# eldenpark/halo2-pse

Hardware: AMD Instinct MI355X
Metric: bn254_msm_g1_adds_per_sec (higher is better)
Workload: dtype u32x8 (256-bit Montgomery integers)

## Files before the change

halo2-pse_amd/__init__.py:

```python
import ctypes
import os
import subprocess

import numpy as np

_HERE = os.path.dirname(os.path.abspath(__file__))
LIB_PATH = os.environ.get("HALO2_HIP_LIB") or os.path.join(_HERE, "libhalo2hip.so")
HEADER_PATH = os.path.join(os.path.dirname(_HERE), "include", "halo2hip.h")

_lib = None


class H2HipError(RuntimeError):
    pass


def build(force=False, jobs=4):
    args = ["make", "-C", _HERE, "-j%d" % jobs]
    if force:
        args.append("-B")
    subprocess.check_call(args, stdout=subprocess.DEVNULL)
    return LIB_PATH


# ... 1140 lines not shown
                                                         ctypes.c_uint32(domain.extended_k), _p(domain.extended_omega), _p(domain.g_coset),
                                                         _p(domain.g_coset_inv), ctypes.c_uint32(blinding_factors), _dptr(d_l0), _dptr(d_l_last),
                                                         _dptr(d_l_active_row), _stream()), "h2hip_key_lagrange_columns_bn254_device")


def set_keygen_group(group_bytes=0):
    _check(lib().h2hip_debug_set_keygen_group(ctypes.c_uint64(group_bytes)), "h2hip_debug_set_keygen_group")


def gen_scalars_device(seed, n, start=0, device="cuda"):
    import torch
    out = torch.empty((n, 4), dtype=torch.int64, device=device)
    _check(lib().h2hip_gen_scalars_device(ctypes.c_uint64(seed), ctypes.c_uint64(start), ctypes.c_size_t(n), _dptr(out), _stream()),
           "h2hip_gen_scalars_device")
    return out


def gen_points_device(seed, n, start=0, device="cuda"):
    import torch
    out = torch.empty((n, 8), dtype=torch.int64, device=device)
    _check(lib().h2hip_gen_points_device(ctypes.c_uint64(seed), ctypes.c_uint64(start), ctypes.c_size_t(n), _dptr(out), _stream()),
           "h2hip_gen_points_device")
    return out


def to_numpy_u64(t):
    return t.detach().cpu().numpy().view(np.uint64)


def set_msm_window(c):
    _check(lib().h2hip_set_msm_window(ctypes.c_uint32(c)), "h2hip_set_msm_window")


def get_msm_window(n):
    return int(lib().h2hip_get_msm_window(n))


def get_msm_window_fixed_base(n):
    return int(lib().h2hip_get_msm_window_fixed_base(n))


def msm_min_n():
    return int(lib().h2hip_msm_min_n())


def ntt_min_log_n():
    return int(lib().h2hip_ntt_min_log_n())


def lazy_pin_after():
    return int(lib().h2hip_lazy_pin_after())


def profile_enable(on=True):
    _check(lib().h2hip_profile_enable(int(on)), "h2hip_profile_enable")


def profile_reset():
    _check(lib().h2hip_profile_reset(), "h2hip_profile_reset")


def profile_get(stage):
    ms = ctypes.c_double(0)
    cnt = ctypes.c_uint64(0)
    _check(lib().h2hip_profile_get(stage.encode(), ctypes.byref(ms), ctypes.byref(cnt)), "h2hip_profile_get")
    return ms.value, cnt.value
# ... 1 lines not shown
```

halo2-pse_amd/csrc/engine.h:

```cpp
#pragma once
#include <hip/hip_runtime.h>
#include <stdint.h>
#include <stdio.h>
#include <string.h>

#include <map>
#include <mutex>
#include <shared_mutex>
#include <string>
#include <vector>

#include "../../include/halo2hip.h"
#include "ecu.h"

namespace h2 {

void set_error(const char* fmt, ...);

#define H2_CHECK(expr)                                                                             \
    do {                                                                                           \
        hipError_t _e = (expr);                                                                    \
        if (_e != hipSuccess) {                                                                    \
            h2::set_error("%s:%d: %s -> %s", __FILE__, __LINE__, #expr, hipGetErrorString(_e));    \
            return 2;                                                                              \
// ... 321 lines not shown
int kzg_setup_device(Ctx* c, uint32_t k, const Fe& s, Affine* d_g, Affine* d_gl, hipStream_t stream);

const Fe* pinned_column_lookup(Ctx* c, const uint64_t* h_col, size_t elems);

void evalh_debug_set_max_local_slots(uint32_t v);
void evalh_debug_set_lookup_group_bytes(uint64_t v);
int evalh_debug_compile_stats(const h2hip_graph* g, uint32_t* n_ops, uint32_t* n_slots);
int evalh_debug_program_muls(const h2hip_graph* g, uint32_t* n_mul);
void evalh_debug_set_codegen(int mode, uint32_t max_ops);
void evalh_debug_codegen_stats(uint64_t out[5]);
int evalh_debug_codegen_source(const h2hip_graph* g, char* buf, size_t cap, size_t* len, int compile, double* seconds, size_t* code_bytes);
void evalh_modules_free(Ctx* c);
void evalh_rtc_shutdown();
int evaluate_h_validate(const h2hip_evalh_desc* d, const void* values);
int evaluate_h_host(Ctx* c, const h2hip_evalh_desc* d, uint64_t* values, bool dev, hipStream_t s);
int lookup_compress_validate(uint32_t n_fixed, uint32_t n_advice, uint32_t n_instance, uint32_t n_challenges, const h2hip_graph* graphs,
                             size_t n_graphs);
int lookup_compress_device(Ctx* c, uint32_t k, const Fe* const* fixed, uint32_t n_fixed, const Fe* const* advice, uint32_t n_advice,
                           const Fe* const* instance, uint32_t n_instance, const uint64_t* challenges, uint32_t n_challenges,
                           const uint64_t theta[4], const h2hip_graph* graphs, size_t n_graphs, Fe* const* out, hipStream_t s);
int check_gates_validate(uint32_t n_fixed, uint32_t n_advice, uint32_t n_instance, uint32_t n_challenges, const h2hip_graph* graphs,
                         size_t n_graphs);
int check_gates_enqueue(Ctx* c, uint32_t k, const Fe* const* fixed, uint32_t n_fixed, const Fe* const* advice, uint32_t n_advice,
                        const Fe* const* instance, uint32_t n_instance, const uint64_t* challenges, uint32_t n_challenges,
                        const h2hip_graph* graphs, size_t n_graphs, uint64_t* d_mask, uint32_t words, hipStream_t s);

void msm_set_fuse_small(bool on);
void msm_set_window(uint32_t c);
void msm_set_max_chunk(size_t m);
void msm_set_stream(uint32_t chunks, double ratio, size_t min_n);
size_t msm_debug_ladder(size_t n, uint32_t chunks, double ratio, bool with_bases, size_t* out, size_t cap);
void msm_set_heavy_div(size_t d);
void msm_set_bin_entries(size_t d);
void msm_set_split_records(bool on);
void msm_set_bucket_order(int local);
void msm_set_quad_tail(bool on);
void msm_set_split_buckets(bool on);
void msm_set_plane_tail(bool on);
void msm_set_fuse_limits(size_t entries, size_t max_n);
void msm_set_rowcol(uint64_t lanes, uint32_t flavour);
void msm_set_reserved_cus(uint32_t k);
uint32_t msm_get_reserved_cus();
uint32_t msm_get_window(size_t n);
int msm_device(Ctx* c, const Fe* d_scalars, const Affine* d_bases, size_t n, XYZZ* h_out, hipStream_t s, const MsmTable* tab = nullptr);
int msm_batch_device(Ctx* c, const Fe* const* scalars, bool scalars_on_host, const Affine* d_bases, size_t n, size_t count, XYZZ* h_out,
                     hipStream_t s, const MsmTable* tab = nullptr, const Affine* h_bases = nullptr);
uint32_t msm_table_window(size_t n);
int msm_table_build(Ctx* c, const Affine* d_points, size_t n, uint32_t cw, Affine* d_table, hipStream_t s);

}
```

halo2-pse_amd/csrc/msm.hip:

```cpp
#include <hip/hip_ext.h>
#include <string.h>

#include <atomic>
#include <condition_variable>
#include <thread>
#include <vector>

#include "ecq.h"
#include "engine.h"
#include "host64.h"

namespace h2 {

#define MSM_MAX_C1 1024u
#define MSM_MAX_L 12u
#define MSM_STAGE 16384u
#define MSM_COUNT_TILE 4096u

struct MsmPlan {
    uint32_t c;
    uint32_t W;
    uint32_t q;
    uint32_t cb;
    uint32_t NB;
    uint32_t shared;
    uint32_t heavy_t;
    uint32_t chunk;
};

template <class F>
__device__ __forceinline__ void for_each_digit(const Fe& s, uint32_t c, uint32_t q, uint32_t W, F&& f) {
    uint64_t buf = 0;
    uint32_t nb = 0, w = 0, carry = 0;
    uint32_t width = q ? c : c - 1;
    auto emit = [&]() {
        uint32_t d = ((uint32_t)buf & ((1u << width) - 1)) + carry;
        uint32_t neg = 0;
        carry = 0;
        if (d > (1u << (width - 1))) {
            d = (1u << width) - d;
            neg = 1;
            carry = 1;
        }
        if (d) f(w, d - 1, neg);
        w++;
        buf >>= width;
        nb = nb > width ? nb - width : 0;
        width = w < q ? c : c - 1;
    };
#pragma unroll
    for (int limb = 0; limb < 8; limb++) {
        buf |= (uint64_t)s.l[limb] << nb;
        nb += 32;
        while (nb >= width && w < W) emit();
    }
    while (w < W) emit();
}

struct L1Args {
    const Fe* scalars_one;
    const Fe* const* list;
    uint32_t n, c, q, W, cb, L, C1;
    uint32_t shared, stride;
    uint32_t tile;
    uint16_t* tile_hist;
    const uint32_t* tile_off;
    uint2* tmp;
    uint32_t* tmp_e;
    uint16_t* tmp_k;
    const Affine* chk_bases;
    const Affine* chk_samples;
    uint32_t* chk_flag;
    size_t chk_n, chk_total;
};

__device__ __forceinline__ Fe fr_to_canonical(const Fe& x) {
    Fu c32 = fu_zero();
    c32.l[0] = 32;
    return fu_mul_canon<FrU>(fu_slice(x), c32);
}

#define MSM_TCHUNK 64u
#ifndef MSM_SCATTER_XG
#define MSM_SCATTER_XG 4u
#endif

__global__ void __launch_bounds__(256) msm_l1_count_kernel(L1Args a) {
    __shared__ uint32_t lh[MSM_MAX_C1];
    if (a.chk_flag && blockIdx.x == 0 && blockIdx.y == 0 && threadIdx.x < 4 * H2_PIN_SAMPLES) {
        const uint32_t k = threadIdx.x >> 2, part = threadIdx.x & 3;
        const size_t idx = pin_sample_index(a.chk_total, k);
        if (idx < a.chk_n) {
            const uint4 u = reinterpret_cast<const uint4*>(&a.chk_bases[idx])[part], v = reinterpret_cast<const uint4*>(&a.chk_samples[k])[part];
            if (u.x != v.x || u.y != v.y || u.z != v.z || u.w != v.w) atomicOr(a.chk_flag, 1u);
        }
    }
    for (uint32_t b = threadIdx.x; b < a.C1; b += 256) lh[b] = 0;
    __syncthreads();
    const Fe* __restrict__ scalars = a.list ? a.list[blockIdx.y] : a.scalars_one;
    const uint32_t set0 = a.shared ? blockIdx.y : blockIdx.y * a.W;
    for (uint32_t t = threadIdx.x; t < a.tile; t += 256) {
        const uint32_t i = blockIdx.x * a.tile + t;
        if (i < a.n) {
            const Fe sc = fr_to_canonical(scalars[i]);
            for_each_digit(sc, a.c, a.q, a.W, [&](uint32_t w, uint32_t slot, uint32_t) {
                const uint32_t gb = ((set0 + (a.shared ? 0u : w)) << a.cb) | slot;
                atomicAdd(&lh[gb >> a.L], 1u);
            });
        }
    }
    __syncthreads();
    uint16_t* row = a.tile_hist + (size_t)(blockIdx.y * gridDim.x + blockIdx.x) * a.C1;
    for (uint32_t b = threadIdx.x; b < a.C1; b += 256) row[b] = (uint16_t)lh[b];
}

__global__ void __launch_bounds__(256) msm_l1_chunk_kernel(const uint16_t* __restrict__ tile_hist, uint32_t n_tiles, uint32_t C1,
                                                           uint32_t* __restrict__ chunk_sum) {
    const uint32_t b = blockIdx.y * 256 + threadIdx.x;
    if (b >= C1) return;
    const uint32_t t0 = blockIdx.x * MSM_TCHUNK, t1 = t0 + MSM_TCHUNK < n_tiles ? t0 + MSM_TCHUNK : n_tiles;
    uint32_t sum = 0;
#pragma unroll 8
    for (uint32_t t = t0; t < t1; t++) sum += tile_hist[(size_t)t * C1 + b];
    chunk_sum[(size_t)blockIdx.x * C1 + b] = sum;
}

template <int BS>
__device__ __forceinline__ uint32_t block_scan_base(const uint32_t* cnt, uint32_t n, uint32_t per, uint32_t* ps, uint32_t* total) {
    const uint32_t t = threadIdx.x;
    uint32_t sum = 0;
    for (uint32_t j = 0; j < per; j++) {
        const uint32_t k = t * per + j;
        if (k < n) sum += cnt[k];
    }
    uint32_t inc = sum;
#pragma unroll
    for (uint32_t off = 1; off < 64; off <<= 1) {
        const uint32_t up = __shfl_up(inc, off, 64);
        if ((t & 63) >= off) inc += up;
    }
    if ((t & 63) == 63) ps[t >> 6] = inc;
    __syncthreads();
    uint32_t before = 0, all = 0;
#pragma unroll
    for (uint32_t w = 0; w < BS / 64; w++) {
        const uint32_t v = ps[w];
        if (w < (t >> 6)) before += v;
        all += v;
    }
    __syncthreads();
    *total = all;
    return before + inc - sum;
}

template <bool SPLIT>
__global__ void __launch_bounds__(1024) msm_l1_scatter_kernel(L1Args a) {
    __shared__ uint2 stage[MSM_STAGE];
    __shared__ uint32_t cur[MSM_MAX_C1];
    __shared__ uint32_t delta[MSM_MAX_C1];
    __shared__ uint32_t ps[16];
    constexpr uint32_t XG = MSM_SCATTER_XG;
    uint32_t tx = blockIdx.x;
    if (XG && tx < (gridDim.x & ~((8u << XG) - 1))) {
        const uint32_t q = tx >> (3 + XG), r = tx & ((8u << XG) - 1);
        tx = ((q * 8 + (r & 7)) << XG) | (r >> 3);
    }
    const size_t row = (size_t)(blockIdx.y * gridDim.x + tx) * a.C1;
    for (uint32_t b = threadIdx.x; b < a.C1; b += 1024) cur[b] = a.tile_hist[row + b];
    const Fe* __restrict__ scalars = a.list ? a.list[blockIdx.y] : a.scalars_one;
    const uint32_t set0 = a.shared ? blockIdx.y : blockIdx.y * a.W;
    const uint32_t i = tx * a.tile + threadIdx.x;
    const bool live = threadIdx.x < a.tile && i < a.n;
    Fe sc;
    if (live) sc = fr_to_canonical(scalars[i]);
    __syncthreads();
    uint32_t total;
    uint32_t run = block_scan_base<1024>(cur, a.C1, 1, ps, &total);
    if (threadIdx.x < a.C1) {
        const uint32_t b = threadIdx.x;
        delta[b] = a.tile_off[row + b] - run;
        cur[b] = run;
    }
    __syncthreads();
    if (live) {
        for_each_digit(sc, a.c, a.q, a.W, [&](uint32_t w, uint32_t slot, uint32_t neg) {
            const uint32_t gb = ((set0 + (a.shared ? 0u : w)) << a.cb) | slot;
            const uint32_t pos = atomicAdd(&cur[gb >> a.L], 1u);
            stage[pos] = make_uint2((a.shared ? w * a.stride + i : i) | (neg << 31), gb);
        });
    }
    __syncthreads();
    for (uint32_t pos = threadIdx.x; pos < total; pos += 1024) {
        const uint2 e = stage[pos];
        const uint32_t at = pos + delta[e.y >> a.L];
        if (SPLIT) {
            a.tmp_e[at] = e.x;
            a.tmp_k[at] = (uint16_t)(e.y & ((1u << a.L) - 1));
        } else {
            a.tmp[at] = e;
        }
    }
}

__global__ void __launch_bounds__(1024) msm_l1_scan_kernel(uint32_t* __restrict__ chunk_sum, uint32_t n_chunks, uint32_t C1,
                                                           uint32_t* __restrict__ bin_total, uint32_t* __restrict__ zero, uint32_t zero_words) {
    __shared__ uint32_t part_sum[16][64];
    if (blockIdx.x == 0)
        for (uint32_t i = threadIdx.x; i < zero_words; i += 1024) zero[i] = 0;
    const uint32_t lb = threadIdx.x & 63, p = threadIdx.x >> 6, b = blockIdx.x * 64 + lb;
    const uint32_t per = (n_chunks + 15) / 16, c0 = p * per, c1 = c0 + per < n_chunks ? c0 + per : n_chunks;
    uint32_t sum = 0;
    if (b < C1)
        for (uint32_t ch = c0; ch < c1; ch++) sum += chunk_sum[(size_t)ch * C1 + b];
    part_sum[p][lb] = sum;
    __syncthreads();
    uint32_t acc = 0, all = 0;
#pragma unroll
    for (uint32_t q = 0; q < 16; q++) {
        const uint32_t v = part_sum[q][lb];
        if (q < p) acc += v;
        all += v;
    }
    if (b < C1) {
        for (uint32_t ch = c0; ch < c1; ch++) {
            const uint32_t v = chunk_sum[(size_t)ch * C1 + b];
            chunk_sum[(size_t)ch * C1 + b] = acc;
            acc += v;
        }
        if (p == 0) bin_total[b] = all;
    }
}

// ... 4 lines not shown
    const uint32_t per = (C1 + 255) / 256;
    uint32_t total;
    uint32_t run = block_scan_base<256>(bin_total, C1, per, ps, &total);
    for (uint32_t j = 0; j < per; j++) {
        const uint32_t k = threadIdx.x * per + j;
        if (k < C1) {
            cs[k] = run;
            run += bin_total[k];
        }
    }
    __syncthreads();
    const uint32_t b = blockIdx.y * 256 + threadIdx.x;
    if (b >= C1) return;
    if (blockIdx.x == 0) {
        coarse_start[b] = cs[b];
        if (b == 0) coarse_start[C1] = total;
    }
    const uint32_t t0 = blockIdx.x * MSM_TCHUNK, t1 = t0 + MSM_TCHUNK < n_tiles ? t0 + MSM_TCHUNK : n_tiles;
    uint32_t running = cs[b] + chunk_sum[(size_t)blockIdx.x * C1 + b];
#pragma unroll 8
    for (uint32_t t = t0; t < t1; t++) {
        tile_off[(size_t)t * C1 + b] = running;
        running += tile_hist[(size_t)t * C1 + b];
    }
}

__device__ __forceinline__ uint32_t size_class(uint32_t cnt, uint32_t bin_shift) {
    uint32_t b = cnt >> bin_shift;
    return 255u - (b < 255u ? b : 255u);
}

template <bool SPLIT>
__global__ void __launch_bounds__(1024) msm_l2_kernel(const uint2* __restrict__ tmp, const uint32_t* __restrict__ tmp_e, const uint16_t* __restrict__ tmp_k,
                                                      const uint32_t* __restrict__ coarse_start, uint32_t L,
                                                      uint32_t bin_shift, uint32_t* __restrict__ vals, uint32_t* __restrict__ start,
                                                      uint32_t* __restrict__ counts, uint32_t* __restrict__ perm, uint32_t* __restrict__ class_hist) {
    constexpr uint32_t NBMAX = 1u << MSM_MAX_L, EPT = MSM_STAGE / 1024;
    __shared__ uint32_t sval[MSM_STAGE];
    __shared__ uint16_t skey[MSM_STAGE];
    __shared__ uint32_t gpos[NBMAX];
    __shared__ uint32_t tcur[NBMAX];
    __shared__ uint32_t tdelta[NBMAX];
    __shared__ uint32_t ps[16], cls[256];
    const uint32_t nb = 1u << L, t = threadIdx.x, per = (nb + 1023) / 1024;
    const uint32_t cs = coarse_start[blockIdx.x], ce = coarse_start[blockIdx.x + 1];
    const bool single = ce - cs <= MSM_STAGE;
    auto load_tile = [&](uint2 (&e)[EPT], uint32_t first, uint32_t tile_n) {
#pragma unroll
        for (uint32_t j = 0; j < EPT; j++) {
            const uint32_t idx = t + j * 1024;
            if (idx < tile_n) e[j] = SPLIT ? make_uint2(tmp_e[first + idx], tmp_k[first + idx]) : tmp[first + idx];
        }
    };
    auto count_tile = [&](const uint2 (&e)[EPT], uint32_t tile_n) {
#pragma unroll
        for (uint32_t j = 0; j < EPT; j++)
            if (t + j * 1024 < tile_n) atomicAdd(&tcur[e[j].y & (nb - 1)], 1u);
    };
    uint2 e[EPT], e_next[EPT];
    const uint32_t first_n = ce - cs < MSM_STAGE ? ce - cs : MSM_STAGE;
    load_tile(e, cs, first_n);
    for (uint32_t k = t; k < nb; k += 1024) tcur[k] = 0;
    if (t < 256) cls[t] = 0;
    __syncthreads();
    if (single) {
        count_tile(e, first_n);
    } else {
        uint32_t idx = cs + t;
        for (; idx + 7 * 1024 < ce; idx += 8 * 1024) {
            uint32_t key[8];
#pragma unroll
            for (uint32_t j = 0; j < 8; j++) key[j] = SPLIT ? (uint32_t)tmp_k[idx + j * 1024] : tmp[idx + j * 1024].y;
#pragma unroll
            for (uint32_t j = 0; j < 8; j++) atomicAdd(&tcur[key[j] & (nb - 1)], 1u);
        }
        for (; idx < ce; idx += 1024) atomicAdd(&tcur[(SPLIT ? (uint32_t)tmp_k[idx] : tmp[idx].y) & (nb - 1)], 1u);
    }
    __syncthreads();
    uint32_t total;
    uint32_t run = block_scan_base<1024>(tcur, nb, per, ps, &total);
    const uint32_t gb0 = blockIdx.x << L;
    for (uint32_t j = 0; j < per; j++) {
        const uint32_t k = t * per + j;
        if (k < nb) {
            const uint32_t cnt = tcur[k];
            gpos[k] = cs + run;
            start[gb0 + k] = cs + run;
            counts[gb0 + k] = cnt;
            atomicAdd(&cls[size_class(cnt, bin_shift)], 1u);
            run += cnt;
        }
    }
    __syncthreads();
    if (class_hist) {
        if (t < 256 && cls[t]) atomicAdd(&class_hist[t], cls[t]);
    } else {
        uint32_t dummy;
        const uint32_t c0 = block_scan_base<1024>(cls, 256, 1, ps, &dummy);
        if (t < 256) tdelta[t] = c0;
        __syncthreads();
        for (uint32_t j = 0; j < per; j++) {
            const uint32_t k = t * per + j;
            if (k < nb) perm[gb0 + atomicAdd(&tdelta[size_class(tcur[k], bin_shift)], 1u)] = gb0 + k;
        }
        __syncthreads();
    }
    for (uint32_t base = cs; base < ce; base += MSM_STAGE) {
        const uint32_t tile_n = ce - base < MSM_STAGE ? ce - base : MSM_STAGE;
        const uint32_t next = base + MSM_STAGE;
        const uint32_t next_n = next < ce ? (ce - next < MSM_STAGE ? ce - next : MSM_STAGE) : 0;
        if (next_n) load_tile(e_next, next, next_n);
        if (!single) {
            for (uint32_t k = t; k < nb; k += 1024) tcur[k] = 0;
            __syncthreads();
            count_tile(e, tile_n);
            __syncthreads();
        }
        run = block_scan_base<1024>(tcur, nb, per, ps, &total);
        for (uint32_t j = 0; j < per; j++) {
            const uint32_t k = t * per + j;
            if (k < nb) {
                const uint32_t cnt = tcur[k];
                tdelta[k] = gpos[k] - run;
                gpos[k] += cnt;
                tcur[k] = run;
                run += cnt;
            }
        }
        __syncthreads();
#pragma unroll
        for (uint32_t j = 0; j < EPT; j++) {
            const uint32_t idx = t + j * 1024;
            if (idx < tile_n) {
                const uint32_t k = e[j].y & (nb - 1);
                const uint32_t pos = atomicAdd(&tcur[k], 1u);
                sval[pos] = e[j].x;
                skey[pos] = (uint16_t)k;
            }
        }
        __syncthreads();
        for (uint32_t pos = t; pos < tile_n; pos += 1024) vals[pos + tdelta[skey[pos]]] = sval[pos];
        __syncthreads();
#pragma unroll
        for (uint32_t j = 0; j < EPT; j++) e[j] = e_next[j];
    }
}

#define MSM_BS_PER 4u
struct HeavyBucket {
    uint32_t bucket, first_chunk, n_chunks, arrived;
};
struct HeavyChunk {
    uint32_t begin, end, owner;
};

__global__ void __launch_bounds__(1024) msm_bucket_scatter_kernel(const uint32_t* __restrict__ counts, const uint32_t* __restrict__ start, uint32_t n_buckets,
                                                                  uint32_t bin_shift, uint32_t heavy_t, uint32_t chunk, uint32_t* __restrict__ hist,
                                                                  uint32_t* __restrict__ perm, uint32_t* __restrict__ heavy_counts,
                                                                  HeavyBucket* __restrict__ heavy_buckets, HeavyChunk* __restrict__ heavy_chunks) {
    __shared__ uint32_t scan[256], lh[256], lbase[256], ps[16];
    const uint32_t t = threadIdx.x;
    for (uint32_t j = 0; j < MSM_BS_PER; j++) {
        const uint32_t b = (blockIdx.x * 1024 + t) * MSM_BS_PER + j;
        const uint32_t cnt = b < n_buckets ? counts[b] : 0;
        if (cnt > heavy_t) {
            const uint32_t s0 = start[b], e0 = s0 + cnt, nch = (cnt + chunk - 1) / chunk;
            const uint32_t slot = atomicAdd(&heavy_counts[1], nch);
// ... 530 lines not shown

__global__ void __launch_bounds__(256) msm_table_step_kernel(const Affine* __restrict__ prev, XYZZ* __restrict__ out, uint32_t n, uint32_t c) {
    const uint32_t i = blockIdx.x * blockDim.x + threadIdx.x;
    if (i >= n) return;
    const Affine p = prev[i];
    if (affine_is_identity(p)) {
        out[i] = xyzz_identity();
        return;
    }
    XYZZu q = xyzzu_double_affine<FqUA>(fu_from_ext(p.x), fu_from_ext(p.y));
    for (uint32_t k = 1; k < c; k++) q = xyzzu_double(q);
    out[i] = xyzzu_to_ext(q);
}

static uint32_t g_window_override = 0;
static size_t g_heavy_div = 32768;
static size_t g_bin_entries = 8192;
static bool g_split_records = true;
void msm_set_split_records(bool on) { g_split_records = on; }
static uint64_t g_rowcol_lanes = 65536;
static bool g_rowcol_asm = true, g_rowcol_qtree = true;
void msm_set_rowcol(uint64_t lanes, uint32_t flavour) {
    g_rowcol_lanes = lanes ? lanes : 65536;
    g_rowcol_asm = flavour & 1;
    g_rowcol_qtree = flavour & 2;
}
static bool g_split_buckets = true;
void msm_set_split_buckets(bool on) { g_split_buckets = on; }
static bool g_quad_tail = true;
void msm_set_quad_tail(bool on) { g_quad_tail = on; }
static bool g_global_order = true;
void msm_set_bucket_order(int local) { g_global_order = local == 0; }
void msm_set_bin_entries(size_t d) { g_bin_entries = d ? d : 8192; }
void msm_set_heavy_div(size_t d) { g_heavy_div = d ? d : 32768; }
static size_t g_max_chunk = (size_t)1 << 26;
void msm_set_max_chunk(size_t m) { g_max_chunk = m ? m : ((size_t)1 << 26); }
static uint32_t g_reserved_cus = 0;
void msm_set_reserved_cus(uint32_t k) { g_reserved_cus = k; }
uint32_t msm_get_reserved_cus() { return g_reserved_cus; }
void msm_set_window(uint32_t c) { g_window_override = c; }

static uint32_t floor_log2(size_t n) {
    uint32_t lg = 0;
    while (((size_t)1 << (lg + 1)) <= n) lg++;
    return lg;
}

static uint32_t plain_window(size_t n, bool fused) {
    if (g_window_override) return g_window_override;
    const uint32_t lg = floor_log2(n);
    if (fused && lg >= 13 && lg <= 18) return lg <= 13 ? 10 : lg <= 16 ? 12 : lg == 17 ? 13 : 14;
    if (lg <= 8) return 7;
    if (lg <= 12) return 10;
    if (lg <= 14) return 13;
    if (lg <= 17) return 15;
    return 17;
}

static uint32_t normalise_window(uint32_t c) {
    if (c < 2) c = 2;
    if (c > 22) c = 22;
    const uint32_t W = (255 + c - 1) / c;
    return (255 + W - 1) / W;
}

uint32_t msm_table_window(size_t n) {
// ... 23 lines not shown
    p.chunk = 1024;
    return p;
}

uint32_t msm_get_window(size_t n) { return make_plan(n, false, nullptr).c; }

static XYZZ combine_windows(const XYZZ* ws, const MsmPlan& p) {
    h64::P acc = h64::identity();
    for (uint32_t w = p.W; w-- > 0;) {
        const uint32_t width = w < p.q ? p.c : p.c - 1;
        for (uint32_t k = 0; k < width; k++) acc = h64::pdouble(acc);
        h64::padd(acc, h64::from_xyzz(ws[w]));
    }
    return h64::to_xyzz(acc);
}

static inline size_t align_up(size_t x, size_t a) { return (x + a - 1) / a * a; }

static uint32_t bits_of(uint32_t v) {
    uint32_t b = 0;
    while (v) {
        b++;
        v >>= 1;
    }
    return b;
}

struct MsmLayout {
    uint32_t fuse;
    uint32_t n_sets;
    MsmPlan p;
    size_t n, E;
    uint32_t K;
    uint32_t L, C1, bin_shift;
    uint32_t tile, tiles_x, n_tiles, n_tchunks;
    uint32_t split_log;
    uint32_t levels, s, rb, s2, s3;
    size_t max_chunks, max_heavy;
    size_t o_zero, o_zero_end, o_bintot, o_hist, o_hcnt, o_fdone, o_cstart, o_tmp, o_vals, o_start, o_counts, o_perm, o_buckets, o_parts, o_RA, o_CA, o_RR,
        o_RC, o_CR, o_CC, o_sums, o_partials, o_ppart, o_hb, o_hc, o_hs, o_ptrs, o_thist, o_toff, o_chsum, total;
};

static int msm_layout(size_t n, MsmLayout* L, uint32_t fuse, const MsmTable* tab, uint32_t force_c = 0, int force_split = -1) {
    MsmPlan p = make_plan(n, fuse > 1, tab, force_c);
    L->p = p;
    L->n = n;
    L->fuse = fuse;
    L->n_sets = p.shared ? fuse : fuse * p.W;
    L->E = n * p.W * fuse;
    if (L->E >= ((size_t)1 << 31)) {
        set_error("msm: %zu entries exceed the 2^31 limit of one run (window override too small?)", L->E);
        return 1;
    }
    if (p.shared && (uint64_t)p.W * tab->stride >= (1ull << 31)) {
        set_error("msm: fixed-base table index exceeds 31 bits");
        return 1;
    }
    const uint64_t K64 = (uint64_t)L->n_sets << p.cb;
    if (K64 > ((uint64_t)MSM_MAX_C1 << MSM_MAX_L)) {
        set_error("msm: too many buckets (%llu) for one run", (unsigned long long)K64);
        return 1;
    }
    L->K = (uint32_t)K64;
    uint32_t want = 1;
    while (want < MSM_MAX_C1 && (size_t)want * g_bin_entries < L->E) want <<= 1;
    uint32_t Lb = 0;
    while (Lb < p.cb && Lb < MSM_MAX_L && (K64 >> Lb) > want) Lb++;
    while ((K64 >> Lb) > MSM_MAX_C1) {
        if (Lb >= p.cb || Lb >= MSM_MAX_L) {
            set_error("msm: too many bucket sets (%u) for one run", L->n_sets);
            return 1;
        }
        Lb++;
    }
    L->L = Lb;
    L->C1 = (uint32_t)(K64 >> Lb);
    L->tile = (MSM_STAGE / p.W) & ~63u;
    if (L->tile > 1024) L->tile = 1024;
    L->tiles_x = (uint32_t)((n + L->tile - 1) / L->tile);
    L->n_tiles = L->tiles_x * fuse;
    L->n_tchunks = (L->n_tiles + MSM_TCHUNK - 1) / MSM_TCHUNK;
    L->bin_shift = 0;
    const size_t mean_bucket = (p.shared ? n * p.W : n) >> p.cb;
    while ((mean_bucket >> L->bin_shift) > 100) L->bin_shift++;
    L->split_log = 0;
    while (L->split_log < 3 && ((uint64_t)L->K << (L->split_log + 1)) <= (1u << 18) && (mean_bucket >> (L->split_log + 1)) >= 2) L->split_log++;
    if (!g_split_buckets) L->split_log = 0;
    if (force_split >= 0) L->split_log = (uint32_t)force_split;
    L->max_chunks = L->E / p.chunk + L->E / p.heavy_t + 16;
    L->max_heavy = L->E / p.heavy_t + 16;
    const uint32_t cb = p.cb;
    L->levels = cb <= 6 ? 0 : cb <= 12 ? 1 : 2;
    L->s = L->levels ? (cb + 1) / 2 : 0;
    L->rb = cb - L->s;
    L->s2 = L->levels == 2 ? (L->rb + 1) / 2 : 0;
    L->s3 = L->levels == 2 ? (L->s + 1) / 2 : 0;
    size_t off = 0;
    auto carve = [&](size_t bytes) { size_t o = off; off = align_up(off + bytes, 256); return o; };
    const size_t E = L->E;
    const uint32_t K = L->K, ns = L->n_sets;
    L->o_zero = off;
    L->o_hist = carve(512 * 4);
    L->o_hcnt = carve(16);
    L->o_fdone = carve((size_t)MSM_MAX_C1 * 4);
    L->o_zero_end = off;
    L->o_cstart = carve(((size_t)MSM_MAX_C1 + 1) * 4);
    L->o_bintot = carve((size_t)MSM_MAX_C1 * 4);
    L->o_start = carve((size_t)K * 4);
    L->o_counts = carve((size_t)K * 4);
// ... 12 lines not shown
    L->o_ptrs = carve((size_t)fuse * sizeof(void*));
    L->o_thist = carve((size_t)L->n_tiles * L->C1 * 2);
    L->o_toff = carve((size_t)L->n_tiles * L->C1 * 4);
    L->o_chsum = carve((size_t)L->n_tchunks * L->C1 * 4);
    L->o_tmp = carve(E * 8);
    L->o_vals = carve(E * 4);
    L->o_hb = carve(L->max_heavy * sizeof(HeavyBucket));
    L->o_hc = carve(L->max_chunks * sizeof(HeavyChunk));
    L->o_hs = carve(L->max_chunks * sizeof(XYZZu));
    L->total = off;
    return 0;
}

static int msm_stage_a(Ctx* c, const MsmLayout& L, char* base, const Fe* const* d_scalars_list, const MsmTable* tab, hipStream_t s) {
    const MsmPlan& p = L.p;
    const size_t n = L.n;
    uint32_t* cstart = (uint32_t*)(base + L.o_cstart);
    uint32_t *vals = (uint32_t*)(base + L.o_vals), *start = (uint32_t*)(base + L.o_start);
    uint32_t *counts = (uint32_t*)(base + L.o_counts), *perm = (uint32_t*)(base + L.o_perm);
    int t0 = c->timer_begin("msm_digits", s);
    L1Args a;
    a.scalars_one = d_scalars_list[0];
    a.list = nullptr;
    if (L.fuse > 1) {
        int rc = c->stage_h2d(base + L.o_ptrs, d_scalars_list, L.fuse * sizeof(void*), s);
        if (rc) return rc;
        a.list = (const Fe* const*)(base + L.o_ptrs);
    }
    a.n = (uint32_t)n;
    a.c = p.c;
    a.q = p.q;
    a.W = p.W;
    a.cb = p.cb;
    a.L = L.L;
    a.C1 = L.C1;
    a.shared = p.shared;
    a.stride = tab ? (uint32_t)tab->stride : 0;
    a.tile = L.tile;
    a.tile_hist = (uint16_t*)(base + L.o_thist);
    a.tile_off = (const uint32_t*)(base + L.o_toff);
    a.tmp = (uint2*)(base + L.o_tmp);
    a.chk_bases = c->pin_chk.bases;
    a.chk_samples = c->pin_chk.samples;
    a.chk_flag = c->pin_chk.flag;
    a.chk_n = c->pin_chk.n;
    a.chk_total = c->pin_chk.total;
    c->pin_chk = Ctx::PinCheck();
    uint32_t* chsum = (uint32_t*)(base + L.o_chsum);
    const dim3 tiles(L.tiles_x, L.fuse), chunks(L.n_tchunks, (L.C1 + 255) / 256);
    hipLaunchKernelGGL(msm_l1_count_kernel, tiles, dim3(256), 0, s, a);
    H2_CHECK(hipGetLastError());
    c->timer_end(t0, s);
    int t1 = c->timer_begin("msm_sort", s);
    hipLaunchKernelGGL(msm_l1_chunk_kernel, chunks, dim3(256), 0, s, (const uint16_t*)a.tile_hist, L.n_tiles, L.C1, chsum);
    H2_CHECK(hipGetLastError());
    uint32_t* bin_total = (uint32_t*)(base + L.o_bintot);
    hipLaunchKernelGGL(msm_l1_scan_kernel, dim3((L.C1 + 63) / 64), dim3(1024), 0, s, chsum, L.n_tchunks, L.C1, bin_total,
                       (uint32_t*)(base + L.o_zero), (uint32_t)((L.o_zero_end - L.o_zero) / 4));
    H2_CHECK(hipGetLastError());
    hipLaunchKernelGGL(msm_l1_offsets_kernel, chunks, dim3(256), 0, s, (const uint16_t*)a.tile_hist, L.n_tiles, L.C1, (const uint32_t*)chsum,
                       (const uint32_t*)bin_total, cstart, (uint32_t*)(base + L.o_toff));
    H2_CHECK(hipGetLastError());
    const bool split = g_split_records && L.E / L.C1 > MSM_STAGE;
    a.tmp_e = (uint32_t*)(base + L.o_tmp);
    a.tmp_k = (uint16_t*)(base + L.o_tmp + L.E * 4);
    if (split)
        hipLaunchKernelGGL(msm_l1_scatter_kernel<true>, tiles, dim3(1024), 0, s, a);
    else
        hipLaunchKernelGGL(msm_l1_scatter_kernel<false>, tiles, dim3(1024), 0, s, a);
    H2_CHECK(hipGetLastError());
    uint32_t* hist = (uint32_t*)(base + L.o_hist);
    if (split)
        hipLaunchKernelGGL(msm_l2_kernel<true>, dim3(L.C1), dim3(1024), 0, s, (const uint2*)nullptr, (const uint32_t*)a.tmp_e, (const uint16_t*)a.tmp_k, cstart,
                           L.L, L.bin_shift, vals, start, counts, perm, g_global_order ? hist : (uint32_t*)nullptr);
    else
        hipLaunchKernelGGL(msm_l2_kernel<false>, dim3(L.C1), dim3(1024), 0, s, (const uint2*)(base + L.o_tmp), (const uint32_t*)nullptr,
                           (const uint16_t*)nullptr, cstart, L.L, L.bin_shift, vals, start, counts, perm, g_global_order ? hist : (uint32_t*)nullptr);
    H2_CHECK(hipGetLastError());
    hipLaunchKernelGGL(msm_bucket_scatter_kernel, dim3((L.K + 1024 * MSM_BS_PER - 1) / (1024 * MSM_BS_PER)), dim3(1024), 0, s, (const uint32_t*)counts,
                       (const uint32_t*)start, L.K, L.bin_shift, p.heavy_t, p.chunk, hist, g_global_order ? perm : (uint32_t*)nullptr,
                       (uint32_t*)(base + L.o_hcnt), (HeavyBucket*)(base + L.o_hb), (HeavyChunk*)(base + L.o_hc));
    H2_CHECK(hipGetLastError());
    c->timer_end(t1, s);
    return 0;
}

static int msm_stage_b(Ctx* c, const MsmLayout& L, char* base, const Affine* d_points, hipStream_t s, char* bbase = nullptr, bool cont = false,
                       bool combine = true) {
    const MsmPlan& p = L.p;
    if (!bbase) bbase = base;
    uint32_t* vals = (uint32_t*)(base + L.o_vals);
    uint32_t *start = (uint32_t*)(base + L.o_start), *counts = (uint32_t*)(base + L.o_counts), *perm = (uint32_t*)(base + L.o_perm);
    XYZZu* buckets = (XYZZu*)(bbase + L.o_buckets);
    uint32_t* hcnt = (uint32_t*)(base + L.o_hcnt);
    HeavyBucket* hb = (HeavyBucket*)(base + L.o_hb);
    HeavyChunk* hc = (HeavyChunk*)(base + L.o_hc);
    XYZZu* hs = (XYZZu*)(base + L.o_hs);
    int t2 = c->timer_begin("msm_accum", s);
    hipEvent_t ke0 = nullptr, ke1 = nullptr;
    XYZZu* parts = (XYZZu*)(bbase + L.o_parts);
    const uint32_t lanes = L.K << L.split_log;
    const uint32_t cont_u = cont ? 1u : 0u;
    const uint32_t hgrid = (uint32_t)(L.max_chunks < (size_t)c->sm_count ? L.max_chunks : (size_t)c->sm_count);
    const dim3 agrid(hgrid + (lanes + 255) / 256);
    if (c->timer_kernel("msm_accum", &ke0, &ke1) >= 0)
        hipExtLaunchKernelGGL(msm_accum_kernel, agrid, dim3(256), 0, s, ke0, ke1, 0, d_points, (const uint32_t*)vals, (const uint32_t*)start,
                              (const uint32_t*)counts, (const uint32_t*)perm, L.K, L.split_log, p.heavy_t, cont_u, parts, hgrid, (const uint32_t*)hcnt, hb,
                              (const HeavyChunk*)hc, hs);
    else
        hipLaunchKernelGGL(msm_accum_kernel, agrid, dim3(256), 0, s, d_points, (const uint32_t*)vals, (const uint32_t*)start, (const uint32_t*)counts,
// ... 534 lines not shown
            if (rc) return rc;
        }
        for (size_t j = 0; j < count; j++) xyzz_add(h_out[j], part[j]);
    }
    return 0;
}

int msm_device(Ctx* c, const Fe* d_scalars, const Affine* d_bases, size_t n, XYZZ* h_out, hipStream_t s, const MsmTable* tab) {
    return msm_batch_device(c, &d_scalars, false, d_bases, n, 1, h_out, s, tab, nullptr);
}

int msm_table_build(Ctx* c, const Affine* d_points, size_t n, uint32_t cw, Affine* d_table, hipStream_t s) {
    const uint32_t W = (255 + cw - 1) / cw, q = 255 - W * (cw - 1);
    if (d_table != d_points) H2_CHECK(hipMemcpyAsync(d_table, d_points, n * sizeof(Affine), hipMemcpyDeviceToDevice, s));
    const size_t slice = (size_t)1 << 22;
    const size_t m_max = n < slice ? n : slice;
    int rc = c->ecfft_ws.ensure(m_max * sizeof(XYZZ));
    if (rc) return rc;
    if ((rc = c->ws_acquire(s))) return rc;
    WsGuard guard(c, s);
    XYZZ* tmp = (XYZZ*)c->ecfft_ws.p;
    for (uint32_t j = 1; j < W; j++) {
        for (size_t o = 0; o < n; o += slice) {
            const size_t m = n - o < slice ? n - o : slice;
            hipLaunchKernelGGL(msm_table_step_kernel, dim3((uint32_t)((m + 255) / 256)), dim3(256), 0, s, d_table + (size_t)(j - 1) * n + o, tmp,
                               (uint32_t)m, (j - 1) < q ? cw : cw - 1);
            H2_CHECK(hipGetLastError());
            if ((rc = ec_normalize_device(tmp, d_table + (size_t)j * n + o, m, s))) return rc;
        }
    }
    return guard.release();
}

}
```

include/halo2hip_debug.h:

```cpp
#ifndef HALO2HIP_DEBUG_H
#define HALO2HIP_DEBUG_H
#include "halo2hip.h"

#ifdef __cplusplus
extern "C" {
#endif

int h2hip_debug_set_msm_stream(uint32_t chunks, uint32_t ratio_permille, size_t min_n);
size_t h2hip_debug_msm_stream_ladder(size_t n, uint32_t chunks, uint32_t ratio_permille, int with_bases, size_t* sizes, size_t cap);
int h2hip_debug_set_msm_max_chunk(size_t m);
int h2hip_debug_rccl_gather_selftest(const uint64_t* partials_xyz, size_t count, uint64_t* out_xyz);
int h2hip_debug_set_msm_heavy_div(size_t d);
int h2hip_debug_set_g2l_quad(int on);
int h2hip_debug_set_msm_fuse_limits(size_t entries, size_t max_n);
int h2hip_debug_set_msm_rowcol(uint64_t lanes, int use_asm);
int h2hip_debug_set_msm_split_buckets(int on);
int h2hip_debug_set_msm_plane_tail(int on);
int h2hip_debug_set_msm_quad_tail(int on);
int h2hip_debug_set_msm_bucket_order(int local);
int h2hip_debug_set_msm_split_records(int on);
int h2hip_debug_set_msm_bin_entries(size_t d);
int h2hip_debug_set_reserved_cus(uint32_t k);
int h2hip_debug_set_msm_fuse_small(int on);
int h2hip_debug_set_ntt_smax(uint32_t v);
int h2hip_debug_ntt_plan(uint32_t log_n, size_t count, uint32_t radices[4]);
int h2hip_debug_set_lazy_pin(uint32_t after);
int h2hip_debug_set_ntt_two_pass(uint32_t lo, uint32_t hi);
int h2hip_debug_set_ntt_twiddle_budget(uint64_t bytes);
int h2hip_debug_set_ntt_batch_bytes(uint64_t bytes);
int h2hip_debug_set_ntt_two_pass_batch_wgs(uint64_t v);
int h2hip_debug_set_ntt_full_max_log_m(uint32_t v);
int h2hip_debug_set_ntt_fold_tables(int on);
int h2hip_debug_set_ntt_host_batch(uint64_t run_bytes, uint64_t group_bytes);
int h2hip_debug_set_ntt_two_pass_log_j(int v);
int h2hip_debug_set_evalh_max_local_slots(uint32_t v);
int h2hip_debug_set_evalh_lookup_group_bytes(uint64_t v);
int h2hip_debug_evalh_program_muls(const h2hip_graph* g, uint32_t* n_mul);
int h2hip_debug_set_evalh_codegen(int mode, uint32_t max_ops);
int h2hip_debug_evalh_codegen_source(const h2hip_graph* g, char* buf, size_t cap, size_t* len, int compile, double* seconds, size_t* code_bytes);
int h2hip_debug_evalh_codegen_stats(uint64_t out[5]);
int h2hip_debug_evalh_compile_stats(const h2hip_graph* g, uint32_t* n_ops, uint32_t* n_slots);
int h2hip_debug_set_opening_tile(uint32_t rows_per_thread, uint32_t threads_per_tile);
int h2hip_debug_set_lookup_sort(uint32_t lds_keys);
int h2hip_debug_lookup_sort_stats(uint32_t out[2]);
int h2hip_debug_set_keygen_group(uint64_t group_bytes);

#ifdef __cplusplus
}
#endif
#endif
```

Before: 11.59 billion.

## Balance MSM coarse sort bins by expected occupancy instead of power-of-two ranges

Replaces the power-of-two coarse binning in the MSM two-level bucket sort with variable-width bins sized by the expected load of each bucket region: wide and narrow windows, and low and high halves of signed digits. The aim is to even out work across the L2 sort workgroups so a few overloaded bins do not dominate. The always-empty upper half of narrow windows is zero-filled directly. This adds a multiply-shift division per digit key and more complex range decoding. The old scheme stays available behind a debug switch.

```diff
diff --git a/halo2-pse_amd/__init__.py b/halo2-pse_amd/__init__.py
--- a/halo2-pse_amd/__init__.py
+++ b/halo2-pse_amd/__init__.py
@@ -1196,6 +1196,24 @@
     _check(lib().h2hip_set_msm_window(ctypes.c_uint32(c)), "h2hip_set_msm_window")
 
 
+def set_msm_pow2_bins(on):
+    _check(lib().h2hip_debug_set_msm_pow2_bins(ctypes.c_int(1 if on else 0)), "h2hip_debug_set_msm_pow2_bins")
+
+
+def msm_bins(n, count=1, c=0, fixed_base=False):
+    L = lib()
+    L.h2hip_debug_msm_bins.restype = ctypes.c_size_t
+    first = np.zeros(1024, dtype=np.uint32)
+    size = np.zeros(1024, dtype=np.uint32)
+    info = (ctypes.c_uint32 * 6)()
+    bins = L.h2hip_debug_msm_bins(ctypes.c_size_t(n), ctypes.c_size_t(count), ctypes.c_uint32(c), ctypes.c_int(1 if fixed_base else 0), _p(first),
+                                  _p(size), ctypes.c_size_t(1024), info)
+    if bins == 0:
+        raise H2HipError("h2hip_debug_msm_bins: no such run: " + L.h2hip_last_error().decode())
+    keys = ("c", "W", "q", "buckets_per_set", "sets", "pow2")
+    return first[:bins].copy(), size[:bins].copy(), dict(zip(keys, (int(v) for v in info)))
+
+
 def get_msm_window(n):
     return int(lib().h2hip_get_msm_window(n))
 
diff --git a/halo2-pse_amd/csrc/engine.h b/halo2-pse_amd/csrc/engine.h
--- a/halo2-pse_amd/csrc/engine.h
+++ b/halo2-pse_amd/csrc/engine.h
@@ -377,6 +377,7 @@
 size_t msm_debug_ladder(size_t n, uint32_t chunks, double ratio, bool with_bases, size_t* out, size_t cap);
 void msm_set_heavy_div(size_t d);
 void msm_set_bin_entries(size_t d);
+void msm_set_pow2_bins(bool on);
 void msm_set_split_records(bool on);
 void msm_set_bucket_order(int local);
 void msm_set_quad_tail(bool on);
diff --git a/halo2-pse_amd/csrc/msm.hip b/halo2-pse_amd/csrc/msm.hip
--- a/halo2-pse_amd/csrc/msm.hip
+++ b/halo2-pse_amd/csrc/msm.hip
@@ -6,14 +6,14 @@
 #include <thread>
 #include <vector>
 
+#include "../../include/halo2hip_debug.h"
 #include "ecq.h"
 #include "engine.h"
 #include "host64.h"
+#include "msm_bins.h"
 
 namespace h2 {
 
-#define MSM_MAX_C1 1024u
-#define MSM_MAX_L 12u
 #define MSM_STAGE 16384u
 #define MSM_COUNT_TILE 4096u
 
@@ -60,7 +60,8 @@
 struct L1Args {
     const Fe* scalars_one;
     const Fe* const* list;
-    uint32_t n, c, q, W, cb, L, C1;
+    uint32_t n, c, q, W, cb, C1;
+    MsmBins bins;
     uint32_t shared, stride;
     uint32_t tile;
     uint16_t* tile_hist;
@@ -98,14 +99,12 @@
     for (uint32_t b = threadIdx.x; b < a.C1; b += 256) lh[b] = 0;
     __syncthreads();
     const Fe* __restrict__ scalars = a.list ? a.list[blockIdx.y] : a.scalars_one;
-    const uint32_t set0 = a.shared ? blockIdx.y : blockIdx.y * a.W;
     for (uint32_t t = threadIdx.x; t < a.tile; t += 256) {
         const uint32_t i = blockIdx.x * a.tile + t;
         if (i < a.n) {
             const Fe sc = fr_to_canonical(scalars[i]);
             for_each_digit(sc, a.c, a.q, a.W, [&](uint32_t w, uint32_t slot, uint32_t) {
-                const uint32_t gb = ((set0 + (a.shared ? 0u : w)) << a.cb) | slot;
-                atomicAdd(&lh[gb >> a.L], 1u);
+                atomicAdd(&lh[msm_bin_key(a.bins, blockIdx.y, w, slot) >> 16], 1u);
             });
         }
     }
@@ -168,7 +167,6 @@
     const size_t row = (size_t)(blockIdx.y * gridDim.x + tx) * a.C1;
     for (uint32_t b = threadIdx.x; b < a.C1; b += 1024) cur[b] = a.tile_hist[row + b];
     const Fe* __restrict__ scalars = a.list ? a.list[blockIdx.y] : a.scalars_one;
-    const uint32_t set0 = a.shared ? blockIdx.y : blockIdx.y * a.W;
     const uint32_t i = tx * a.tile + threadIdx.x;
     const bool live = threadIdx.x < a.tile && i < a.n;
     Fe sc;
@@ -184,20 +182,20 @@
     __syncthreads();
     if (live) {
         for_each_digit(sc, a.c, a.q, a.W, [&](uint32_t w, uint32_t slot, uint32_t neg) {
-            const uint32_t gb = ((set0 + (a.shared ? 0u : w)) << a.cb) | slot;
-            const uint32_t pos = atomicAdd(&cur[gb >> a.L], 1u);
-            stage[pos] = make_uint2((a.shared ? w * a.stride + i : i) | (neg << 31), gb);
+            const uint32_t bk = msm_bin_key(a.bins, blockIdx.y, w, slot);
+            const uint32_t pos = atomicAdd(&cur[bk >> 16], 1u);
+            stage[pos] = make_uint2((a.shared ? w * a.stride + i : i) | (neg << 31), bk);
         });
     }
     __syncthreads();
     for (uint32_t pos = threadIdx.x; pos < total; pos += 1024) {
         const uint2 e = stage[pos];
-        const uint32_t at = pos + delta[e.y >> a.L];
+        const uint32_t at = pos + delta[e.y >> 16];
         if (SPLIT) {
             a.tmp_e[at] = e.x;
-            a.tmp_k[at] = (uint16_t)(e.y & ((1u << a.L) - 1));
+            a.tmp_k[at] = (uint16_t)e.y;
         } else {
-            a.tmp[at] = e;
+            a.tmp[at] = make_uint2(e.x, e.y & 0xffffu);
         }
     }
 }
@@ -268,7 +266,7 @@
 
 template <bool SPLIT>
 __global__ void __launch_bounds__(1024) msm_l2_kernel(const uint2* __restrict__ tmp, const uint32_t* __restrict__ tmp_e, const uint16_t* __restrict__ tmp_k,
-                                                      const uint32_t* __restrict__ coarse_start, uint32_t L,
+                                                      const uint32_t* __restrict__ coarse_start, MsmBins bins,
                                                       uint32_t bin_shift, uint32_t* __restrict__ vals, uint32_t* __restrict__ start,
                                                       uint32_t* __restrict__ counts, uint32_t* __restrict__ perm, uint32_t* __restrict__ class_hist) {
     constexpr uint32_t NBMAX = 1u << MSM_MAX_L, EPT = MSM_STAGE / 1024;
@@ -278,7 +276,9 @@
     __shared__ uint32_t tcur[NBMAX];
     __shared__ uint32_t tdelta[NBMAX];
     __shared__ uint32_t ps[16], cls[256];
-    const uint32_t nb = 1u << L, t = threadIdx.x, per = (nb + 1023) / 1024;
+    uint32_t gb0, nb, zb0, znb;
+    msm_bin_range(bins, blockIdx.x, &gb0, &nb, &zb0, &znb);
+    const uint32_t t = threadIdx.x, per = (nb + 1023) / 1024;
     const uint32_t cs = coarse_start[blockIdx.x], ce = coarse_start[blockIdx.x + 1];
     const bool single = ce - cs <= MSM_STAGE;
     auto load_tile = [&](uint2 (&e)[EPT], uint32_t first, uint32_t tile_n) {
@@ -291,7 +291,7 @@
     auto count_tile = [&](const uint2 (&e)[EPT], uint32_t tile_n) {
 #pragma unroll
         for (uint32_t j = 0; j < EPT; j++)
-            if (t + j * 1024 < tile_n) atomicAdd(&tcur[e[j].y & (nb - 1)], 1u);
+            if (t + j * 1024 < tile_n) atomicAdd(&tcur[e[j].y], 1u);
     };
     uint2 e[EPT], e_next[EPT];
     const uint32_t first_n = ce - cs < MSM_STAGE ? ce - cs : MSM_STAGE;
@@ -308,14 +308,19 @@
 #pragma unroll
             for (uint32_t j = 0; j < 8; j++) key[j] = SPLIT ? (uint32_t)tmp_k[idx + j * 1024] : tmp[idx + j * 1024].y;
 #pragma unroll
-            for (uint32_t j = 0; j < 8; j++) atomicAdd(&tcur[key[j] & (nb - 1)], 1u);
-        }
-        for (; idx < ce; idx += 1024) atomicAdd(&tcur[(SPLIT ? (uint32_t)tmp_k[idx] : tmp[idx].y) & (nb - 1)], 1u);
+            for (uint32_t j = 0; j < 8; j++) atomicAdd(&tcur[key[j]], 1u);
+        }
+        for (; idx < ce; idx += 1024) atomicAdd(&tcur[SPLIT ? (uint32_t)tmp_k[idx] : tmp[idx].y], 1u);
     }
     __syncthreads();
     uint32_t total;
     uint32_t run = block_scan_base<1024>(tcur, nb, per, ps, &total);
-    const uint32_t gb0 = blockIdx.x << L;
+    for (uint32_t k = t; k < znb; k += 1024) {
+        start[zb0 + k] = cs;
+        counts[zb0 + k] = 0;
+        if (!class_hist) perm[zb0 + k] = zb0 + k;
+    }
+    if (t == 0 && znb) atomicAdd(&cls[size_class(0, bin_shift)], znb);
     for (uint32_t j = 0; j < per; j++) {
         const uint32_t k = t * per + j;
         if (k < nb) {
@@ -368,7 +373,7 @@
         for (uint32_t j = 0; j < EPT; j++) {
             const uint32_t idx = t + j * 1024;
             if (idx < tile_n) {
-                const uint32_t k = e[j].y & (nb - 1);
+                const uint32_t k = e[j].y;
                 const uint32_t pos = atomicAdd(&tcur[k], 1u);
                 sval[pos] = e[j].x;
                 skey[pos] = (uint16_t)k;
@@ -965,6 +970,8 @@
 static bool g_global_order = true;
 void msm_set_bucket_order(int local) { g_global_order = local == 0; }
 void msm_set_bin_entries(size_t d) { g_bin_entries = d ? d : 8192; }
+static bool g_pow2_bins = false;
+void msm_set_pow2_bins(bool on) { g_pow2_bins = on; }
 void msm_set_heavy_div(size_t d) { g_heavy_div = d ? d : 32768; }
 static size_t g_max_chunk = (size_t)1 << 26;
 void msm_set_max_chunk(size_t m) { g_max_chunk = m ? m : ((size_t)1 << 26); }
@@ -1054,7 +1061,8 @@
     MsmPlan p;
     size_t n, E;
     uint32_t K;
-    uint32_t L, C1, bin_shift;
+    uint32_t C1, bin_shift;
+    MsmBins bins;
     uint32_t tile, tiles_x, n_tiles, n_tchunks;
     uint32_t split_log;
     uint32_t levels, s, rb, s2, s3;
@@ -1084,19 +1092,11 @@
         return 1;
     }
     L->K = (uint32_t)K64;
-    uint32_t want = 1;
-    while (want < MSM_MAX_C1 && (size_t)want * g_bin_entries < L->E) want <<= 1;
-    uint32_t Lb = 0;
-    while (Lb < p.cb && Lb < MSM_MAX_L && (K64 >> Lb) > want) Lb++;
-    while ((K64 >> Lb) > MSM_MAX_C1) {
-        if (Lb >= p.cb || Lb >= MSM_MAX_L) {
-            set_error("msm: too many bucket sets (%u) for one run", L->n_sets);
-            return 1;
-        }
-        Lb++;
-    }
-    L->L = Lb;
-    L->C1 = (uint32_t)(K64 >> Lb);
+    if (!msm_plan_bins(&L->bins, p.cb, p.q, p.W, p.shared, fuse, L->E, g_bin_entries, !g_pow2_bins)) {
+        set_error("msm: too many bucket sets (%u) for one run", L->n_sets);
+        return 1;
+    }
+    L->C1 = L->bins.C1;
     L->tile = (MSM_STAGE / p.W) & ~63u;
     if (L->tile > 1024) L->tile = 1024;
     L->tiles_x = (uint32_t)((n + L->tile - 1) / L->tile);
@@ -1175,7 +1175,7 @@
     a.q = p.q;
     a.W = p.W;
     a.cb = p.cb;
-    a.L = L.L;
+    a.bins = L.bins;
     a.C1 = L.C1;
     a.shared = p.shared;
     a.stride = tab ? (uint32_t)tab->stride : 0;
@@ -1215,10 +1215,10 @@
     uint32_t* hist = (uint32_t*)(base + L.o_hist);
     if (split)
         hipLaunchKernelGGL(msm_l2_kernel<true>, dim3(L.C1), dim3(1024), 0, s, (const uint2*)nullptr, (const uint32_t*)a.tmp_e, (const uint16_t*)a.tmp_k, cstart,
-                           L.L, L.bin_shift, vals, start, counts, perm, g_global_order ? hist : (uint32_t*)nullptr);
+                           L.bins, L.bin_shift, vals, start, counts, perm, g_global_order ? hist : (uint32_t*)nullptr);
     else
         hipLaunchKernelGGL(msm_l2_kernel<false>, dim3(L.C1), dim3(1024), 0, s, (const uint2*)(base + L.o_tmp), (const uint32_t*)nullptr,
-                           (const uint16_t*)nullptr, cstart, L.L, L.bin_shift, vals, start, counts, perm, g_global_order ? hist : (uint32_t*)nullptr);
+                           (const uint16_t*)nullptr, cstart, L.bins, L.bin_shift, vals, start, counts, perm, g_global_order ? hist : (uint32_t*)nullptr);
     H2_CHECK(hipGetLastError());
     hipLaunchKernelGGL(msm_bucket_scatter_kernel, dim3((L.K + 1024 * MSM_BS_PER - 1) / (1024 * MSM_BS_PER)), dim3(1024), 0, s, (const uint32_t*)counts,
                        (const uint32_t*)start, L.K, L.bin_shift, p.heavy_t, p.chunk, hist, g_global_order ? perm : (uint32_t*)nullptr,
@@ -1819,4 +1819,33 @@
     return guard.release();
 }
 
-}
+static size_t msm_debug_bins(size_t n, size_t count, uint32_t c, bool fixed_base, uint32_t* first, uint32_t* size, size_t cap, uint32_t info[6]) {
+    if (!n || !count || count > MSM_MAX_C1) return 0;
+    MsmTable tab;
+    tab.c = c ? normalise_window(c) : msm_table_window(n);
+    tab.stride = n;
+    MsmLayout L;
+    if (msm_layout(n, &L, (uint32_t)count, fixed_base ? &tab : nullptr, fixed_base ? 0 : c)) return 0;
+    for (uint32_t b = 0; b < L.C1 && b < cap; b++) {
+        uint32_t f, nb, zf, znb;
+        msm_bin_range(L.bins, b, &f, &nb, &zf, &znb);
+        if (first) first[b] = f;
+        if (size) size[b] = nb;
+    }
+    if (info) {
+        const uint32_t v[6] = {L.p.c, L.p.W, L.p.q, L.p.NB, L.n_sets, L.bins.pow2};
+        memcpy(info, v, sizeof(v));
+    }
+    return L.C1;
+}
+
+}
+
+extern "C" int h2hip_debug_set_msm_pow2_bins(int on) {
+    h2::msm_set_pow2_bins(on != 0);
+    return 0;
+}
+
+extern "C" size_t h2hip_debug_msm_bins(size_t n, size_t count, uint32_t c, int fixed_base, uint32_t* first, uint32_t* size, size_t cap, uint32_t info[6]) {
+    return h2::msm_debug_bins(n, count, c, fixed_base != 0, first, size, cap, info);
+}
diff --git a/halo2-pse_amd/csrc/msm_bins.h b/halo2-pse_amd/csrc/msm_bins.h
--- /dev/null
+++ b/halo2-pse_amd/csrc/msm_bins.h
@@ -0,0 +1,142 @@
+#pragma once
+#include <stdint.h>
+
+#if defined(__HIPCC__)
+#define H2_BINS_FN __host__ __device__ __forceinline__
+#else
+#define H2_BINS_FN inline
+#endif
+
+namespace h2 {
+
+#define MSM_MAX_C1 1024u
+#define MSM_MAX_L 12u
+
+struct MsmBinRegion {
+    uint32_t bin0;
+    uint32_t b0;
+    uint32_t width;
+    uint32_t mul;
+};
+
+struct MsmBins {
+    uint32_t pow2;
+    uint32_t L;
+    uint32_t cb, q, W, shared;
+    uint32_t half;
+    uint32_t bins_wide, bins_narrow, bins_msm;
+    MsmBinRegion r[3];
+    uint32_t nbins[3];
+    uint32_t C1;
+    uint32_t target;
+};
+
+H2_BINS_FN uint32_t msm_bin_div(uint32_t x, uint32_t width, uint32_t mul) { return width == 1 ? x : (uint32_t)(((uint64_t)x * mul) >> 32); }
+
+H2_BINS_FN uint32_t msm_bin_key(const MsmBins& B, uint32_t y, uint32_t w, uint32_t slot) {
+    if (B.pow2) {
+        const uint32_t gb = ((B.shared ? y : y * B.W + w) << B.cb) | slot;
+        return ((gb >> B.L) << 16) | (gb & ((1u << B.L) - 1));
+    }
+    const bool narrow = !B.shared && w >= B.q, hi = slot >= B.half;
+    uint32_t bin = y * B.bins_msm;
+    if (!B.shared) bin += narrow ? B.q * B.bins_wide + (w - B.q) * B.bins_narrow : w * B.bins_wide;
+    const uint32_t w0 = B.r[0].width, w1 = B.r[1].width, w2 = B.r[2].width, m0 = B.r[0].mul, m1 = B.r[1].mul, m2 = B.r[2].mul;
+    const bool up = hi && !narrow;
+    const uint32_t width = narrow ? w2 : up ? w1 : w0, mul = narrow ? m2 : up ? m1 : m0;
+    const uint32_t x = slot - (up ? B.half : 0u), j = msm_bin_div(x, width, mul);
+    return ((bin + (up ? B.r[1].bin0 : 0u) + j) << 16) | (x - j * width);
+}
+
+H2_BINS_FN void msm_bin_range(const MsmBins& B, uint32_t bin, uint32_t* first, uint32_t* nb, uint32_t* zfirst, uint32_t* znb) {
+    *zfirst = *znb = 0;
+    if (B.pow2) {
+        *first = bin << B.L;
+        *nb = 1u << B.L;
+        return;
+    }
+    const uint32_t y = bin / B.bins_msm;
+    uint32_t r = bin % B.bins_msm, set = y, k = 0;
+    if (!B.shared) {
+        const uint32_t wide = B.q * B.bins_wide;
+        if (r < wide) {
+            set = y * B.W + r / B.bins_wide;
+            r %= B.bins_wide;
+        } else {
+            r -= wide;
+            set = y * B.W + B.q + r / B.bins_narrow;
+            r %= B.bins_narrow;
+            k = 2;
+        }
+    }
+    if (k == 0 && r >= B.r[1].bin0) k = 1;
+    const MsmBinRegion g = k == 0 ? B.r[0] : k == 1 ? B.r[1] : B.r[2];
+    const uint32_t rel = (r - g.bin0) * g.width;
+    *first = (set << B.cb) + g.b0 + rel;
+    *nb = B.half - rel < g.width ? B.half - rel : g.width;
+    if (k == 2) {
+        *zfirst = *first + B.half;
+        *znb = *nb;
+    }
+}
+
+inline bool msm_plan_bins_pow2(MsmBins* B, uint32_t n_sets, uint64_t E, uint64_t bin_entries) {
+    const uint64_t K = (uint64_t)n_sets << B->cb;
+    uint32_t want = 1;
+    while (want < MSM_MAX_C1 && (uint64_t)want * bin_entries < E) want <<= 1;
+    uint32_t Lb = 0;
+    while (Lb < B->cb && Lb < MSM_MAX_L && (K >> Lb) > want) Lb++;
+    while ((K >> Lb) > MSM_MAX_C1) {
+        if (Lb >= B->cb || Lb >= MSM_MAX_L) return false;
+        Lb++;
+    }
+    B->pow2 = 1;
+    B->L = Lb;
+    B->C1 = (uint32_t)(K >> Lb);
+    return true;
+}
+
+inline bool msm_plan_bins(MsmBins* B, uint32_t cb, uint32_t q, uint32_t W, uint32_t shared, uint32_t fuse, uint64_t E, uint64_t bin_entries,
+                          bool balanced) {
+    *B = MsmBins();
+    B->cb = cb;
+    B->q = q;
+    B->W = W;
+    B->shared = shared;
+    B->half = cb ? 1u << (cb - 1) : 0;
+    const uint32_t n_sets = shared ? fuse : fuse * W;
+    if (balanced && cb >= 1 && B->half <= (1u << 20)) {
+        const uint32_t weight[3] = {shared ? 2 * W - q : 1u, shared ? q : 1u, 2u};
+        const uint32_t sets[3] = {shared ? 1u : q, shared ? 1u : q, shared ? 0u : W - q};
+        const uint32_t min_b = (B->half + (1u << MSM_MAX_L) - 1) >> MSM_MAX_L, max_b = B->half;
+        uint32_t want = 1;
+        while (want < MSM_MAX_C1 && (uint64_t)want * bin_entries < E) want <<= 1;
+        for (uint32_t T = want / fuse ? want / fuse : 1; T >= 1; T--) {
+            uint32_t per_msm = 0, width[3], nb[3];
+            for (uint32_t k = 0; k < 3; k++) {
+                uint32_t m = (2 * T * weight[k] + 2 * W) / (4 * W);
+                m = m < min_b ? min_b : m > max_b ? max_b : m;
+                width[k] = (B->half + m - 1) / m;
+                nb[k] = (B->half + width[k] - 1) / width[k];
+                per_msm += sets[k] * nb[k];
+            }
+            if ((uint64_t)per_msm * fuse > MSM_MAX_C1) continue;
+            for (uint32_t k = 0; k < 3; k++) {
+                B->r[k].bin0 = k == 1 ? nb[0] : 0;
+                B->r[k].b0 = k == 1 ? B->half : 0;
+                B->r[k].width = width[k];
+                B->r[k].mul = width[k] > 1 ? (uint32_t)((((uint64_t)1 << 32) + width[k] - 1) / width[k]) : 0;
+                B->nbins[k] = nb[k];
+            }
+            B->bins_wide = nb[0] + nb[1];
+            B->bins_narrow = shared ? 0 : nb[2];
+            B->bins_msm = per_msm;
+            B->C1 = per_msm * fuse;
+            B->target = T;
+            return true;
+        }
+    }
+    return msm_plan_bins_pow2(B, n_sets, E, bin_entries);
+}
+
+}
diff --git a/include/halo2hip_debug.h b/include/halo2hip_debug.h
--- a/include/halo2hip_debug.h
+++ b/include/halo2hip_debug.h
@@ -20,6 +20,8 @@
 int h2hip_debug_set_msm_bucket_order(int local);
 int h2hip_debug_set_msm_split_records(int on);
 int h2hip_debug_set_msm_bin_entries(size_t d);
+int h2hip_debug_set_msm_pow2_bins(int on);
+size_t h2hip_debug_msm_bins(size_t n, size_t count, uint32_t c, int fixed_base, uint32_t* first, uint32_t* size, size_t cap, uint32_t info[6]);
 int h2hip_debug_set_reserved_cus(uint32_t k);
 int h2hip_debug_set_msm_fuse_small(int on);
 int h2hip_debug_set_ntt_smax(uint32_t v);
```

After: 11.44 billion. 0.987x the previous value.
